# aticejiang/MLAgg-UNet

Measured on AMD Instinct MI355X. Metric: images/sec (train step) MLAgg-UNet-2D 256x256 bs10, higher is better.
Workload: dtype f32

## Files before the change

### mlagg-unet_amd/csrc/linear_x3.hip

```cpp
#include <hip/hip_runtime.h>

#include <cstdlib>

#include "mlagg_hip.h"
#include "prof.h"
#include "bf16x3.h"

namespace {

typedef float f32x16 __attribute__((ext_vector_type(16)));
typedef unsigned int u32x4 __attribute__((ext_vector_type(4)));

constexpr int KC = 32;
constexpr int PITCH = KC + 8;

struct X3Geom {
    int M, N, K, Kp, x_stride, y_stride, pre_stride;
};

__device__ __forceinline__ float gelu_f(float x) { return 0.5f * x * (1.f + erff(x * 0.70710678118654752f)); }
__device__ __forceinline__ float gelu_grad_f(float x)
{
    return 0.5f * (1.f + erff(x * 0.70710678118654752f)) + x * 0.3989422804014327f * __expf(-0.5f * x * x);
}

constexpr int APITCH = KC + 4;

template <int NW, int TN, int EPI>
__global__ void __launch_bounds__(64 * NW)
linear_x3_kernel(const float *__restrict__ X, const unsigned short *__restrict__ Wimg, const float *__restrict__ bias,
                 float *__restrict__ Y, float *__restrict__ Y2, const float *__restrict__ PRE, X3Geom g)
{
    constexpr int NT = 64 * NW;
    constexpr int BN = 32 * TN;
    constexpr int NITEM = 3 * BN * 4;
    constexpr int NLD = (NITEM + NT - 1) / NT;
    constexpr int BM = 32 * NW;
    constexpr int NLA = BM * 8 / NT;
    __shared__ float sA[BM * APITCH];
    __shared__ unsigned short sB[3 * BN * PITCH];
    const int tid = threadIdx.x, lane = tid & 63, wave = tid >> 6;
    const int col = lane & 31, kh = lane >> 5;
    const int m0 = blockIdx.x * BM, n0 = blockIdx.y * BN;

    f32x16 acc[TN];
#pragma unroll
    for (int t = 0; t < TN; ++t)
#pragma unroll
        for (int r = 0; r < 16; ++r) acc[t][r] = 0.f;

    const size_t piece_elems = (size_t)g.N * g.Kp;
    unsigned src_off[NLD], dst_off[NLD];
#pragma unroll
    for (int j = 0; j < NLD; ++j) {
        const int i = min(tid + NT * j, NITEM - 1);
        const int piece = i / (BN * 4), rem = i - piece * (BN * 4), row = rem >> 2, seg = rem & 3;
        src_off[j] = (unsigned)(piece * piece_elems + (size_t)min(n0 + row, g.N - 1) * g.Kp + 8 * seg);
        dst_off[j] = (unsigned)(piece * BN * PITCH + row * PITCH + 8 * seg);
    }
    const float *xa[NLA];
#pragma unroll
    for (int i = 0; i < NLA; ++i) xa[i] = X + (size_t)min(m0 + (tid >> 3) + (NT / 8) * i, g.M - 1) * g.x_stride + 4 * (tid & 7);
    struct Regs {
        u32x4 rb[NLD];
        float4 ra[NLA];
        bool ok;
    };
    auto fetch = [&](Regs &R, int kc) {
#pragma unroll
        for (int j = 0; j < NLD; ++j) R.rb[j] = *reinterpret_cast<const u32x4 *>(Wimg + (size_t)src_off[j] + kc);
        R.ok = kc + 4 * (tid & 7) < g.K;
#pragma unroll
        for (int i = 0; i < NLA; ++i) R.ra[i] = *reinterpret_cast<const float4 *>(xa[i] + (R.ok ? kc : 0));
    };
    auto stage = [&](const Regs &R) {
#pragma unroll
        for (int j = 0; j < NLD; ++j) *reinterpret_cast<u32x4 *>(&sB[dst_off[j]]) = R.rb[j];
#pragma unroll
        for (int i = 0; i < NLA; ++i)
            *reinterpret_cast<float4 *>(sA + ((tid >> 3) + (NT / 8) * i) * APITCH + 4 * (tid & 7)) =
                make_float4(R.ok ? R.ra[i].x : 0.f, R.ok ? R.ra[i].y : 0.f, R.ok ? R.ra[i].z : 0.f, R.ok ? R.ra[i].w : 0.f);
    };
    auto multiply = [&]() {
#pragma unroll
        for (int p = 0; p < 2; ++p) {
            const float *ap = sA + (32 * wave + col) * APITCH + 16 * p + 8 * kh;
            const float4 lo4 = *reinterpret_cast<const float4 *>(ap), hi4 = *reinterpret_cast<const float4 *>(ap + 4);
            uint4 aq[3];
            bf16x3::split3(lo4.x, lo4.y, aq[0].x, aq[1].x, aq[2].x);
            bf16x3::split3(lo4.z, lo4.w, aq[0].y, aq[1].y, aq[2].y);
            bf16x3::split3(hi4.x, hi4.y, aq[0].z, aq[1].z, aq[2].z);
            bf16x3::split3(hi4.z, hi4.w, aq[0].w, aq[1].w, aq[2].w);
            uint4 b[TN][3];
#pragma unroll
            for (int t = 0; t < TN; ++t)
#pragma unroll
                for (int q = 0; q < 3; ++q)
                    b[t][q] = *reinterpret_cast<const uint4 *>(sB + q * BN * PITCH + (32 * t + col) * PITCH + 16 * p + 8 * kh);
#pragma unroll
            for (int term = 0; term < 6; ++term)
#pragma unroll
                for (int t = 0; t < TN; ++t)
                    acc[t] = bf16x3::mfma(aq[bf16x3::kTermA[term]], b[t][bf16x3::kTermB[term]], acc[t]);
        }
    };

    const int nchunks = g.Kp / KC;
    Regs R;
    fetch(R, 0);
    for (int c = 0; c < nchunks; ++c) {
        __syncthreads();
        stage(R);
        __syncthreads();
        if (c + 1 < nchunks) fetch(R, (c + 1) * KC);
        multiply();
    }

    const bool rows_full = m0 + 32 * NW <= g.M;
    const int mrow = m0 + 32 * wave + 4 * kh;
    float *yb = Y + (size_t)mrow * g.y_stride;
    float *y2b = EPI == 1 ? Y2 + (size_t)mrow * g.y_stride : nullptr;
    const float *pb = EPI == 2 ? PRE + (size_t)mrow * g.pre_stride : nullptr;
#pragma unroll
    for (int t = 0; t < TN; ++t) {
        const int n = n0 + 32 * t + col;
        if (n0 + 32 * t >= g.N) break;
        const float bv = (EPI != 2 && bias) ? bias[min(n, g.N - 1)] : 0.f;
        if (n < g.N) {
            if (rows_full) {
                float pre[16];
                if (EPI == 2) {
#pragma unroll
                    for (int r = 0; r < 16; ++r) pre[r] = pb[((r & 3) + 8 * (r >> 2)) * g.pre_stride + n];
                }
#pragma unroll
                for (int r = 0; r < 16; ++r) {
                    const int ro = ((r & 3) + 8 * (r >> 2)) * g.y_stride + n;
                    const float v = acc[t][r] + bv;
                    if (EPI == 2) {
                        yb[ro] = acc[t][r] * gelu_grad_f(pre[r]);
                    } else {
                        yb[ro] = v;
                        if (EPI == 1) y2b[ro] = gelu_f(v);
                    }
                }
            } else {
#pragma unroll
                for (int r = 0; r < 16; ++r) {
                    const int dr = (r & 3) + 8 * (r >> 2);
                    if (mrow + dr < g.M) {
                        const float v = acc[t][r] + bv;
                        if (EPI == 2) {
                            yb[dr * g.y_stride + n] = acc[t][r] * gelu_grad_f(pb[dr * g.pre_stride + n]);
                        } else {
                            yb[dr * g.y_stride + n] = v;
                            if (EPI == 1) y2b[dr * g.y_stride + n] = gelu_f(v);
                        }
                    }
                }
            }
        }
    }
}

struct ImgJob {
    const float *w;
    unsigned short *img;
    unsigned short *imgT;
    int N, K, w_stride, pad;
};

__device__ __forceinline__ void image_tile(const ImgJob &jb, int tile)
{
    __shared__ unsigned short tl[3][32][34];
    const int N = jb.N, K = jb.K;
    const int Kp = (K + 31) & ~31, Np = (N + 31) & ~31;
    const int tk = Kp / 32;
    const int n0 = (tile / tk) * 32, k0 = (tile % tk) * 32;
    const int r = threadIdx.x >> 3, c4 = (threadIdx.x & 7) * 4;
    const int n = n0 + r, k = k0 + c4;
    float v[4] = {0.f, 0.f, 0.f, 0.f};
    if (n < N) {
#pragma unroll
        for (int j = 0; j < 4; ++j)
            if (k + j < K) v[j] = jb.w[(size_t)n * jb.w_stride + k + j];
    }
    unsigned h0, m0, l0, h1, m1, l1;
    bf16x3::split3(v[0], v[1], h0, m0, l0);
    bf16x3::split3(v[2], v[3], h1, m1, l1);
    const unsigned pc[3][2] = {{h0, h1}, {m0, m1}, {l0, l1}};
    if (jb.img && n < N) {
#pragma unroll
        for (int q = 0; q < 3; ++q)
            *reinterpret_cast<uint2 *>(jb.img + ((size_t)q * N + n) * Kp + k) = make_uint2(pc[q][0], pc[q][1]);
    }
    if (jb.imgT) {
#pragma unroll
        for (int q = 0; q < 3; ++q) {
            tl[q][r][c4] = (unsigned short)(pc[q][0] & 0xffffu);
            tl[q][r][c4 + 1] = (unsigned short)(pc[q][0] >> 16);
            tl[q][r][c4 + 2] = (unsigned short)(pc[q][1] & 0xffffu);
            tl[q][r][c4 + 3] = (unsigned short)(pc[q][1] >> 16);
        }
        __syncthreads();
        const int kk = k0 + r;
        if (kk < K) {
#pragma unroll
            for (int q = 0; q < 3; ++q) {
                const unsigned a = tl[q][c4][r] | ((unsigned)tl[q][c4 + 1][r] << 16);
                const unsigned b = tl[q][c4 + 2][r] | ((unsigned)tl[q][c4 + 3][r] << 16);
                *reinterpret_cast<uint2 *>(jb.imgT + ((size_t)q * K + kk) * Np + n0 + c4) = make_uint2(a, b);
            }
        }
    }
}

__global__ void __launch_bounds__(256) weight_image_kernel(ImgJob jb)
{
    image_tile(jb, blockIdx.x);
}

__global__ void __launch_bounds__(256) weight_images_kernel(const ImgJob *__restrict__ jobs)
{
    const ImgJob jb = jobs[blockIdx.y];
    const int tiles = (((jb.K + 31) & ~31) / 32) * ((jb.N + 31) / 32);
    if ((int)blockIdx.x >= tiles) return;
    image_tile(jb, blockIdx.x);
}

template <int NW, int TN>
int launch_x3(const float *x, const unsigned short *img, const float *bias, float *y, float *y2, const float *pre, const X3Geom &g,
              int epilogue, hipStream_t st)
{
    const dim3 grid((g.M + 32 * NW - 1) / (32 * NW), (g.N + 32 * TN - 1) / (32 * TN)), block(64 * NW);
    if (grid.y > 65535) return MLAGG_E_UNSUPPORTED;
    switch (epilogue) {
    case 0: hipLaunchKernelGGL((linear_x3_kernel<NW, TN, 0>), grid, block, 0, st, x, img, bias, y, y2, pre, g); break;
    case 1: hipLaunchKernelGGL((linear_x3_kernel<NW, TN, 1>), grid, block, 0, st, x, img, bias, y, y2, pre, g); break;
    case 2: hipLaunchKernelGGL((linear_x3_kernel<NW, TN, 2>), grid, block, 0, st, x, img, bias, y, y2, pre, g); break;
    default: return MLAGG_E_UNSUPPORTED;
    }
    return (int)hipGetLastError();
}

}

extern "C" size_t mlagg_weight_image_bytes(int rows, int cols)
{
    return (size_t)3 * rows * ((cols + 31) & ~31) * sizeof(unsigned short);
}

extern "C" int mlagg_weight_image(const float *w, int w_stride, void *img, void *img_t, int N, int K, void *stream)
{
    if (!w || (!img && !img_t)) return MLAGG_E_NULLPTR;
    if (N <= 0 || K <= 0 || w_stride < K) return MLAGG_E_UNSUPPORTED;
    ImgJob jb{w, static_cast<unsigned short *>(img), static_cast<unsigned short *>(img_t), N, K, w_stride, 0};
    const int tiles = (((K + 31) & ~31) / 32) * ((N + 31) / 32);
    hipLaunchKernelGGL(weight_image_kernel, dim3(tiles), dim3(256), 0, static_cast<hipStream_t>(stream), jb);
    return (int)hipGetLastError();
}

extern "C" int mlagg_weight_images(const void *jobs, int n_jobs, int max_tiles, void *stream)
{
    if (!jobs) return MLAGG_E_NULLPTR;
    if (n_jobs <= 0 || n_jobs > 65535 || max_tiles <= 0) return MLAGG_E_UNSUPPORTED;
    hipLaunchKernelGGL(weight_images_kernel, dim3(max_tiles, n_jobs), dim3(256), 0, static_cast<hipStream_t>(stream),
                       static_cast<const ImgJob *>(jobs));
    return (int)hipGetLastError();
}

extern "C" int mlagg_linear_x3_supported(int M, int N, int K)
{
    return M > 0 && N > 0 && K > 0 && (K & 7) == 0 && (size_t)3 * N * ((K + 31) & ~31) < (1ull << 32);
}

extern "C" int mlagg_linear_x3(const float *x, int x_stride, const void *w_image, const float *bias, float *y, int y_stride,
                               float *y_act, const float *pre, int pre_stride, int M, int N, int K, int epilogue, void *stream)
{
    if (!x || !w_image || !y) return MLAGG_E_NULLPTR;
    if (!mlagg_linear_x3_supported(M, N, K) || (x_stride & 3) || x_stride < K || y_stride < N) return MLAGG_E_UNSUPPORTED;
    if ((epilogue == 1 && !y_act) || (epilogue == 2 && (!pre || pre_stride < N))) return MLAGG_E_NULLPTR;
    X3Geom g{M, N, K, (K + 31) & ~31, x_stride, y_stride, pre_stride};
    hipStream_t st = static_cast<hipStream_t>(stream);
    MLAGG_TIMED(K_LINEAR_FWD, st);
    const unsigned short *img = static_cast<const unsigned short *>(w_image);
    static const int forced = [] { const char *e = getenv("MLAGG_X3_TILE"); return e ? atoi(e) : 0; }();
    int nw = M <= 1024 ? 2 : 4, tn = 2;
    if (N % 96 == 0 && (long)((M + 127) / 128) * (N / 96) >= 1024) tn = 3;
    if (forced) { nw = forced / 10; tn = forced % 10; }
    if (nw == 4 && tn == 3) return launch_x3<4, 3>(x, img, bias, y, y_act, pre, g, epilogue, st);
    if (nw == 4 && tn == 2) return launch_x3<4, 2>(x, img, bias, y, y_act, pre, g, epilogue, st);
    if (nw == 2 && tn == 3) return launch_x3<2, 3>(x, img, bias, y, y_act, pre, g, epilogue, st);
    if (nw == 2 && tn == 2) return launch_x3<2, 2>(x, img, bias, y, y_act, pre, g, epilogue, st);
    return MLAGG_E_UNSUPPORTED;
}
```

Measured before the change: 298.0.

## Add persistent multi-stage LDS-DMA ring kernel for mid-size bf16x3 linears

Adds a persistent GEMM kernel for the split-bf16 (bf16x3) linear layer. It uses a three-stage LDS ring filled by global_load_lds_dwordx4 direct-to-LDS loads, XOR-swizzled LDS layouts, XCD-aware tile assignment, and vmcnt-based waits, so global loads overlap with MFMA work. The kernel is selected by default for M in 2048..16384 with K>=384, and a 2D wave arrangement is used for larger tile counts. The cost is inline assembly, occupancy queries, and a new correctness surface around the waitcnt logic and bounds clamping.

```diff
diff --git a/mlagg-unet_amd/csrc/linear_x3.hip b/mlagg-unet_amd/csrc/linear_x3.hip
--- a/mlagg-unet_amd/csrc/linear_x3.hip
+++ b/mlagg-unet_amd/csrc/linear_x3.hip
@@ -1,5 +1,6 @@
 #include <hip/hip_runtime.h>
 
+#include <algorithm>
 #include <cstdlib>
 
 #include "mlagg_hip.h"
@@ -25,6 +26,56 @@
 }
 
 constexpr int APITCH = KC + 4;
+
+template <int TN, int EPI, bool BV>
+__device__ __forceinline__ void x3_store(const f32x16 (&acc)[TN], const float *__restrict__ bias, const float *bv, const X3Geom &g,
+                                         float *__restrict__ Y, float *__restrict__ Y2, const float *__restrict__ PRE, int mrow, int n0,
+                                         int col, bool rows_full)
+{
+    float *yb = Y + (size_t)mrow * g.y_stride;
+    float *y2b = EPI == 1 ? Y2 + (size_t)mrow * g.y_stride : nullptr;
+    const float *pb = EPI == 2 ? PRE + (size_t)mrow * g.pre_stride : nullptr;
+#pragma unroll
+    for (int t = 0; t < TN; ++t) {
+        const int n = n0 + 32 * t + col;
+        if (n0 + 32 * t >= g.N) break;
+        const float bvt = BV ? bv[t] : (EPI != 2 && bias) ? bias[min(n, g.N - 1)] : 0.f;
+        if (n < g.N) {
+            if (rows_full) {
+                float pre[16];
+                if (EPI == 2) {
+#pragma unroll
+                    for (int r = 0; r < 16; ++r) pre[r] = pb[((r & 3) + 8 * (r >> 2)) * g.pre_stride + n];
+                }
+#pragma unroll
+                for (int r = 0; r < 16; ++r) {
+                    const int ro = ((r & 3) + 8 * (r >> 2)) * g.y_stride + n;
+                    const float v = acc[t][r] + bvt;
+                    if (EPI == 2) {
+                        yb[ro] = acc[t][r] * gelu_grad_f(pre[r]);
+                    } else {
+                        yb[ro] = v;
+                        if (EPI == 1) y2b[ro] = gelu_f(v);
+                    }
+                }
+            } else {
+#pragma unroll
+                for (int r = 0; r < 16; ++r) {
+                    const int dr = (r & 3) + 8 * (r >> 2);
+                    if (mrow + dr < g.M) {
+                        const float v = acc[t][r] + bvt;
+                        if (EPI == 2) {
+                            yb[dr * g.y_stride + n] = acc[t][r] * gelu_grad_f(pb[dr * g.pre_stride + n]);
+                        } else {
+                            yb[dr * g.y_stride + n] = v;
+                            if (EPI == 1) y2b[dr * g.y_stride + n] = gelu_f(v);
+                        }
+                    }
+                }
+            }
+        }
+    }
+}
 
 template <int NW, int TN, int EPI>
 __global__ void __launch_bounds__(64 * NW)
@@ -116,50 +167,155 @@
         multiply();
     }
 
-    const bool rows_full = m0 + 32 * NW <= g.M;
-    const int mrow = m0 + 32 * wave + 4 * kh;
-    float *yb = Y + (size_t)mrow * g.y_stride;
-    float *y2b = EPI == 1 ? Y2 + (size_t)mrow * g.y_stride : nullptr;
-    const float *pb = EPI == 2 ? PRE + (size_t)mrow * g.pre_stride : nullptr;
-#pragma unroll
-    for (int t = 0; t < TN; ++t) {
-        const int n = n0 + 32 * t + col;
-        if (n0 + 32 * t >= g.N) break;
-        const float bv = (EPI != 2 && bias) ? bias[min(n, g.N - 1)] : 0.f;
-        if (n < g.N) {
-            if (rows_full) {
-                float pre[16];
-                if (EPI == 2) {
-#pragma unroll
-                    for (int r = 0; r < 16; ++r) pre[r] = pb[((r & 3) + 8 * (r >> 2)) * g.pre_stride + n];
-                }
-#pragma unroll
-                for (int r = 0; r < 16; ++r) {
-                    const int ro = ((r & 3) + 8 * (r >> 2)) * g.y_stride + n;
-                    const float v = acc[t][r] + bv;
-                    if (EPI == 2) {
-                        yb[ro] = acc[t][r] * gelu_grad_f(pre[r]);
-                    } else {
-                        yb[ro] = v;
-                        if (EPI == 1) y2b[ro] = gelu_f(v);
-                    }
-                }
-            } else {
-#pragma unroll
-                for (int r = 0; r < 16; ++r) {
-                    const int dr = (r & 3) + 8 * (r >> 2);
-                    if (mrow + dr < g.M) {
-                        const float v = acc[t][r] + bv;
-                        if (EPI == 2) {
-                            yb[dr * g.y_stride + n] = acc[t][r] * gelu_grad_f(pb[dr * g.pre_stride + n]);
-                        } else {
-                            yb[dr * g.y_stride + n] = v;
-                            if (EPI == 1) y2b[dr * g.y_stride + n] = gelu_f(v);
-                        }
-                    }
-                }
+    x3_store<TN, EPI, false>(acc, bias, nullptr, g, Y, Y2, PRE, m0 + 32 * wave + 4 * kh, n0, col, m0 + 32 * NW <= g.M);
+}
+
+template <int N>
+__device__ __forceinline__ void wait_vmcnt()
+{
+    asm volatile("s_waitcnt vmcnt(%0)" ::"n"(N) : "memory");
+}
+
+__device__ __forceinline__ void dma16(const void *src, unsigned lds_dst)
+{
+    asm volatile("s_nop 0\n\tglobal_load_lds_dwordx4 %0, off" ::"v"(src), "{m0}"(lds_dst) : "memory");
+}
+
+template <int S, int WM, int WN, int TN>
+struct RingShape {
+    static constexpr int NWV = WM * WN, NT = 64 * NWV, BM = 32 * WM, BN = 32 * TN * WN;
+    static constexpr int A_BYTES = BM * 128, B_BYTES = 3 * BN * 64, STAGE = A_BYTES + B_BYTES, LDS = S * STAGE;
+    static constexpr int GA = BM * 8 / 64 / NWV;
+    static constexpr int GB = 3 * BN * 4 / 64 / NWV;
+    static_assert((BM * 8) % (64 * NWV) == 0 && (3 * BN * 4) % (64 * NWV) == 0, "DMA pieces must split evenly over the waves");
+    static_assert(BN % 16 == 0 && S >= 3 && (S - 2) * (GA + GB) <= 63, "ring shape");
+};
+
+template <int S, int WM, int WN, int TN, int EPI>
+__global__ void __launch_bounds__(64 * WM * WN)
+linear_x3_ring_kernel(const float *__restrict__ X, const unsigned short *__restrict__ Wimg, const float *__restrict__ bias,
+                      float *__restrict__ Y, float *__restrict__ Y2, const float *__restrict__ PRE, X3Geom g, int ntn, int ntiles)
+{
+    using RS = RingShape<S, WM, WN, TN>;
+    constexpr int BM = RS::BM, BN = RS::BN, GA = RS::GA, GB = RS::GB, STAGE = RS::STAGE, A_BYTES = RS::A_BYTES;
+    constexpr int GW = GA + GB;
+    __shared__ __attribute__((aligned(1024))) unsigned char lds[RS::LDS];
+    const int lane = threadIdx.x & 63, wave = __builtin_amdgcn_readfirstlane(threadIdx.x >> 6);
+    const int col = lane & 31, kh = lane >> 5;
+    const int wm = wave % WM, wn = wave / WM;
+
+    const int G = gridDim.x, b = blockIdx.x, xcd = b % 8, q8 = G / 8, r8 = G % 8;
+    const int wg = (xcd < r8 ? xcd * (q8 + 1) : r8 * (q8 + 1) + (xcd - r8) * q8) + b / 8;
+    const int nch = g.Kp / KC;
+    const int total = (ntiles - wg + G - 1) / G * nch;
+
+    int a_row[GA], a_col[GA];
+#pragma unroll
+    for (int j = 0; j < GA; ++j) {
+        const int rr = (wave * GA + j) * 8 + (lane >> 3);
+        a_row[j] = rr;
+        a_col[j] = 4 * ((lane & 7) ^ ((rr >> 1) & 7));
+    }
+    int b_row[GB];
+    unsigned b_col[GB];
+#pragma unroll
+    for (int j = 0; j < GB; ++j) {
+        const int rr = (wave * GB + j) * 16 + (lane >> 2), piece = rr / BN, r = rr - piece * BN;
+        b_row[j] = r;
+        b_col[j] = (unsigned)(piece * (size_t)g.N * g.Kp) + 8 * ((lane & 3) ^ ((r >> 2) & 3));
+    }
+
+    int ld_tile = wg, ld_k = 0, ld_slot = 0;
+    const float *a_src[GA];
+    unsigned b_src[GB];
+    auto tile_bases = [&]() {
+        const int m0 = (ld_tile / ntn) * BM, n0 = (ld_tile % ntn) * BN;
+#pragma unroll
+        for (int j = 0; j < GA; ++j) a_src[j] = X + (size_t)min(m0 + a_row[j], g.M - 1) * g.x_stride;
+#pragma unroll
+        for (int j = 0; j < GB; ++j) b_src[j] = b_col[j] + (unsigned)min(n0 + b_row[j], g.N - 1) * g.Kp;
+    };
+    const unsigned lds_base = (unsigned)(size_t)(__attribute__((address_space(3))) unsigned char *)lds;
+    auto issue = [&]() {
+        const unsigned st = lds_base + ld_slot * STAGE;
+#pragma unroll
+        for (int j = 0; j < GA; ++j)
+            dma16(a_src[j] + (ld_k + a_col[j] < g.K ? ld_k + a_col[j] : 0), st + (wave * GA + j) * 1024);
+#pragma unroll
+        for (int j = 0; j < GB; ++j) dma16(Wimg + b_src[j] + ld_k, st + A_BYTES + (wave * GB + j) * 1024);
+        ld_k += KC;
+        ld_slot = ld_slot == S - 1 ? 0 : ld_slot + 1;
+        if (ld_k == g.Kp) {
+            ld_k = 0;
+            ld_tile += G;
+            tile_bases();
+        }
+    };
+
+    tile_bases();
+#pragma unroll
+    for (int i = 0; i < S - 1; ++i)
+        if (i < total) issue();
+
+    f32x16 acc[TN];
+#pragma unroll
+    for (int t = 0; t < TN; ++t)
+#pragma unroll
+        for (int r = 0; r < 16; ++r) acc[t][r] = 0.f;
+
+    const int a_rd = (32 * wm + col) * 128, a_x = (col >> 1) & 7;
+    const int b_rd = A_BYTES + (32 * TN * wn + col) * 64, b_x = (col >> 2) & 3;
+    int slot = 0, it = 0;
+#pragma unroll 1
+    for (int tile = wg; tile < ntiles; tile += G) {
+#pragma unroll 1
+        for (int c = 0; c < nch; ++c, ++it) {
+            const int younger = total - 1 - it;
+            if (S >= 4 && younger >= 2) wait_vmcnt<(S >= 4 ? 2 : 0) * GW>();
+            else if (younger >= 1) wait_vmcnt<GW>();
+            else wait_vmcnt<0>();
+            asm volatile("s_waitcnt lgkmcnt(0)" ::: "memory");
+            __builtin_amdgcn_s_barrier();
+            asm volatile("" ::: "memory");
+            if (it + S - 1 < total) issue();
+
+            const unsigned char *st = lds + slot * STAGE;
+#pragma unroll
+            for (int p = 0; p < 2; ++p) {
+                const int s0 = 4 * p + 2 * kh;
+                const float4 lo4 = *reinterpret_cast<const float4 *>(st + a_rd + 16 * (s0 ^ a_x));
+                const float4 hi4 = *reinterpret_cast<const float4 *>(st + a_rd + 16 * ((s0 + 1) ^ a_x));
+                uint4 aq[3];
+                bf16x3::split3(lo4.x, lo4.y, aq[0].x, aq[1].x, aq[2].x);
+                bf16x3::split3(lo4.z, lo4.w, aq[0].y, aq[1].y, aq[2].y);
+                bf16x3::split3(hi4.x, hi4.y, aq[0].z, aq[1].z, aq[2].z);
+                bf16x3::split3(hi4.z, hi4.w, aq[0].w, aq[1].w, aq[2].w);
+                uint4 bq[TN][3];
+#pragma unroll
+                for (int t = 0; t < TN; ++t)
+#pragma unroll
+                    for (int q = 0; q < 3; ++q)
+                        bq[t][q] = *reinterpret_cast<const uint4 *>(st + b_rd + (q * BN + 32 * t) * 64 + 16 * ((2 * p + kh) ^ b_x));
+#pragma unroll
+                for (int term = 0; term < 6; ++term)
+#pragma unroll
+                    for (int t = 0; t < TN; ++t)
+                        acc[t] = bf16x3::mfma(aq[bf16x3::kTermA[term]], bq[t][bf16x3::kTermB[term]], acc[t]);
             }
-        }
+            slot = slot == S - 1 ? 0 : slot + 1;
+        }
+        const int m0 = (tile / ntn) * BM, n0 = (tile % ntn) * BN + 32 * TN * wn;
+        float bv[TN];
+#pragma unroll
+        for (int t = 0; t < TN; ++t) {
+            bv[t] = (EPI != 2 && bias) ? bias[min(n0 + 32 * t + col, g.N - 1)] : 0.f;
+            asm volatile("" ::"v"(bv[t]));
+        }
+        x3_store<TN, EPI, true>(acc, nullptr, bv, g, Y, Y2, PRE, m0 + 32 * wm + 4 * kh, n0, col, m0 + 32 * wm + 32 <= g.M);
+#pragma unroll
+        for (int t = 0; t < TN; ++t)
+#pragma unroll
+            for (int r = 0; r < 16; ++r) acc[t][r] = 0.f;
     }
 }
 
@@ -243,6 +399,35 @@
     return (int)hipGetLastError();
 }
 
+template <int S, int WM, int WN, int TN>
+int launch_x3_ring(const float *x, const unsigned short *img, const float *bias, float *y, float *y2, const float *pre, const X3Geom &g,
+                   int epilogue, hipStream_t st)
+{
+    using RS = RingShape<S, WM, WN, TN>;
+    static int resident[64];
+    int dev = 0;
+    if (hipGetDevice(&dev) != hipSuccess || dev < 0 || dev >= 64) return MLAGG_E_UNSUPPORTED;
+    if (!resident[dev]) {
+        int cus = 0, per_cu = 0;
+        if (hipDeviceGetAttribute(&cus, hipDeviceAttributeMultiprocessorCount, dev) != hipSuccess ||
+            hipOccupancyMaxActiveBlocksPerMultiprocessor(&per_cu, linear_x3_ring_kernel<S, WM, WN, TN, 0>, RS::NT, 0) != hipSuccess)
+            return MLAGG_E_UNSUPPORTED;
+        resident[dev] = cus * (per_cu > 0 ? per_cu : 1);
+    }
+    const int ntn = (g.N + RS::BN - 1) / RS::BN;
+    const long ntiles = (long)((g.M + RS::BM - 1) / RS::BM) * ntn;
+    if (ntiles > (1l << 30)) return MLAGG_E_UNSUPPORTED;
+    const dim3 grid((unsigned)std::min<long>(ntiles, resident[dev])), block(RS::NT);
+    const int nt = (int)ntiles;
+    switch (epilogue) {
+    case 0: hipLaunchKernelGGL((linear_x3_ring_kernel<S, WM, WN, TN, 0>), grid, block, 0, st, x, img, bias, y, y2, pre, g, ntn, nt); break;
+    case 1: hipLaunchKernelGGL((linear_x3_ring_kernel<S, WM, WN, TN, 1>), grid, block, 0, st, x, img, bias, y, y2, pre, g, ntn, nt); break;
+    case 2: hipLaunchKernelGGL((linear_x3_ring_kernel<S, WM, WN, TN, 2>), grid, block, 0, st, x, img, bias, y, y2, pre, g, ntn, nt); break;
+    default: return MLAGG_E_UNSUPPORTED;
+    }
+    return (int)hipGetLastError();
+}
+
 }
 
 extern "C" size_t mlagg_weight_image_bytes(int rows, int cols)
@@ -284,13 +469,23 @@
     hipStream_t st = static_cast<hipStream_t>(stream);
     MLAGG_TIMED(K_LINEAR_FWD, st);
     const unsigned short *img = static_cast<const unsigned short *>(w_image);
-    static const int forced = [] { const char *e = getenv("MLAGG_X3_TILE"); return e ? atoi(e) : 0; }();
-    int nw = M <= 1024 ? 2 : 4, tn = 2;
-    if (N % 96 == 0 && (long)((M + 127) / 128) * (N / 96) >= 1024) tn = 3;
-    if (forced) { nw = forced / 10; tn = forced % 10; }
-    if (nw == 4 && tn == 3) return launch_x3<4, 3>(x, img, bias, y, y_act, pre, g, epilogue, st);
-    if (nw == 4 && tn == 2) return launch_x3<4, 2>(x, img, bias, y, y_act, pre, g, epilogue, st);
-    if (nw == 2 && tn == 3) return launch_x3<2, 3>(x, img, bias, y, y_act, pre, g, epilogue, st);
-    if (nw == 2 && tn == 2) return launch_x3<2, 2>(x, img, bias, y, y_act, pre, g, epilogue, st);
+    const char *forced = getenv("MLAGG_X3_TILE");
+    int code = forced ? atoi(forced) : 0;
+    if (!code) {
+        if (M >= 2048 && M <= 16384 && K >= 384) {
+            code = (long)((M + 127) / 128) * ((N + 127) / 128) >= 180 ? 3422 : 3412;
+        } else {
+            code = (M <= 1024 ? 20 : 40) + ((N % 96 == 0 && (long)((M + 127) / 128) * (N / 96) >= 1024) ? 3 : 2);
+        }
+    }
+    switch (code) {
+    case 43: return launch_x3<4, 3>(x, img, bias, y, y_act, pre, g, epilogue, st);
+    case 42: return launch_x3<4, 2>(x, img, bias, y, y_act, pre, g, epilogue, st);
+    case 23: return launch_x3<2, 3>(x, img, bias, y, y_act, pre, g, epilogue, st);
+    case 22: return launch_x3<2, 2>(x, img, bias, y, y_act, pre, g, epilogue, st);
+    case 3414: return launch_x3_ring<3, 4, 1, 4>(x, img, bias, y, y_act, pre, g, epilogue, st);
+    case 3412: return launch_x3_ring<3, 4, 1, 2>(x, img, bias, y, y_act, pre, g, epilogue, st);
+    case 3422: return launch_x3_ring<3, 4, 2, 2>(x, img, bias, y, y_act, pre, g, epilogue, st);
+    }
     return MLAGG_E_UNSUPPORTED;
 }
```

Measured after the change: 299.4, median of 6. Within noise of the previous version (+0.5%).
